# biointec/columba

Measured on AMD Instinct MI355X. Metric: reads/sec (150bp, k=4 edit, human ref), higher is better.
Workload: dtype u64; 1 GPU; synthetic human-like reference 3000 Mbp (GRCh38 is not available offline), 10000000 x 150 bp reads per GPU, k=4 edit distance, ALL mode, multiple_opt schemes with dynamic selection, dynamic partitioning, in-text switch 4, SA sparseness 4; reads_per_gpu=10000000, read_len=150, k=4, genome_bp=3000000000, index_bytes_hbm=24766778153, parallelism=read-shard x1, occurrences=33415092

## Files before the change

### columba_amd/csrc/columba_amd.hip

```cpp
#include "../../include/columba_amd.h"
#include "host_sam.hpp"
#include "host_schemes.hpp"
#include "kernels.hpp"
#include "dev_sam.hpp"

#include <chrono>
#include <cstring>
#include <functional>
#include <memory>
#include <mutex>
#include <thread>
#include <string>
#include <vector>

using namespace cmb;

static thread_local std::string g_err;
static int fail(int code, const std::string& msg) {
    g_err = msg;
    return code;
}
namespace cmb {
int failWith(int code, const std::string& msg) { return fail(code, msg); }
}
// ... 551 lines not shown

struct KernelTime {
    const char* name;
    float ms;
};

struct cmb_batch {
    cmb_index* ix = nullptr;
    uint32_t k = 0, nReads = 0, maxLen = 0, gw = 0;
    uint32_t minLen = 0;
    int metric = 1;
    DevStrategyK hostStrat{};
    bool wide = false;
    bool wideEdit = false;
    bool geoX = false;
    bool noSmallMatrix = false;
    DevStrategyKT<MAXP_WIDE> hostStratW{};
    DevBuf<DevStrategyKT<MAXP_WIDE>> stratW;
    DevBuf<PartOutT<MAXP_WIDE>> partsW;
    uint32_t sNumParts = 0, sPartition = 0, sNSchemes = 0, sMaxSearches = 0;
    hipStream_t stream = nullptr;
    DevBuf<uint8_t> reads, seq;
    DevBuf<uint32_t> rec;
    DevBuf<uint4> exr;
    DevBuf<uint8_t> psel;
    uint32_t recW = 0;
    DevBuf<uint64_t> offs;
    DevBuf<uint32_t> G;
    DevBuf<uint4> mfull;
    DevBuf<DevStrategyK> strat;
    DevBuf<uint4> bfsQ[2], bfsEv[2], bfsF, bfsC, bfsA;
    DevBuf<uint32_t> bfsCnt;
    DevBuf<unsigned long long> bfsBlockCnt;
    size_t bfsQCap = 0, bfsEvCap = 0, bfsFCap = 0, bfsCCap = 0, bfsACap = 0;
    DevBuf<uint4> nvQ[2];
    DevBuf<uint32_t> nvCnt;
    size_t nvQCap = 0;
    bool hasNaive = false;
    DevBuf<PartOut> parts;
    DevBuf<DfsTask> dfs;
    DevBuf<uint64_t> vW;
    DevBuf<uint4> tbq;
    DevBuf<uint8_t> dpSlab;
    DevBuf<uint32_t> dpList, dpWork;
    DevBuf<uint4> items;
    DevBuf<FMOccRec> fm, fmUniq;
    DevBuf<TextOccRec> text;
// ... 159 lines not shown
            minLen = std::min<uint32_t>(minLen, (uint32_t)(offs[i + 1] - offs[i]));
        }
        b->minLen = n_reads ? minLen : 0u;
        if (maxLen > (uint32_t)MAX_READ)
            return fail(CMB_ERR_UNSUPPORTED, "reads longer than " + std::to_string(MAX_READ) + " are not supported");
        maxLen = (maxLen + 15u) & ~15u;
        b->maxLen = maxLen;
        b->gw = gWords(maxLen);
        b->hostOffs.assign(offs, offs + n_reads + 1);
        HIPCHK(hipStreamCreateWithFlags(&b->stream, hipStreamNonBlocking));
        b->reads.uploadPadded((const uint8_t*)seqs, offs[n_reads], 64);
        b->offs.upload(offs, n_reads + 1);
        b->seq.alloc((size_t)2 * n_reads * maxLen);
        b->G.alloc((size_t)n_reads * 8 * b->gw);
        b->recW = ((1 + 2 * ((maxLen + 31) / 32)) + 3) / 4 * 4;
        b->rec.alloc((size_t)2 * n_reads * b->recW);
        if (b->wide) {
            b->stratW.upload(&b->hostStratW, 1);
            b->partsW.alloc((size_t)2 * n_reads);
        } else {
            b->strat.upload(&b->hostStrat, 1);
            b->parts.alloc((size_t)2 * n_reads);
        }
        b->dfs.alloc((size_t)n_reads * 2 + 4096);
        b->items.alloc((size_t)n_reads * 64 + 4096);
        b->fm.alloc((size_t)n_reads * 8 + 4096);
        b->text.alloc((size_t)n_reads * 48 + 4096);
        b->cnt.alloc(8);
        b->counters.alloc(CMB_CNT_MAX);
        *out = b.release();
        return CMB_OK;
    } catch (const std::exception& e) {
        return fail(CMB_ERR_DEVICE, e.what());
    }
}

namespace {

struct Timer {
    hipStream_t s;
    hipEvent_t a, b;
    std::vector<KernelTime>& out;
    Timer(hipStream_t st, std::vector<KernelTime>& o) : s(st), out(o) {
        (void)hipEventCreate(&a);
        (void)hipEventCreate(&b);
    }
    ~Timer() {
        (void)hipEventDestroy(a);
// ... 203 lines not shown
            HIPCHK(hipStreamSynchronize(s));
            memset(hcnt, 0, sizeof(hcnt));
            hcnt[0] = (uint32_t)b->presetItems.size();
            q.items = b->items.p;
            q.itemCap = (uint32_t)std::min<size_t>(b->items.n, 0xFFFFFFF0u);
        }
        int bfsAttempts = 0;
        for (int attempt = 0; !preset; attempt++) {
            HIPCHK(hipMemsetAsync(b->cnt.p, 0, 8 * sizeof(uint32_t), s));
            if (attempt) {
                HIPCHK(hipMemsetAsync(b->counters.p, 0, CMB_CNT_MAX * sizeof(unsigned long long), s));
            }
            q.items = b->items.p;
            q.itemCap = (uint32_t)std::min<size_t>(b->items.n, 0xFFFFFFF0u);
            q.fm = b->fm.p;
            q.fmCap = (uint32_t)std::min<size_t>(b->fm.n, 0xFFFFFFF0u);
            q.text = b->text.p;
            q.textCap = (uint32_t)std::min<size_t>(b->text.n, 0xFFFFFFF0u);
            const uint32_t dfsCap = (uint32_t)std::min<size_t>(b->dfs.n, 0xFFFFFFF0u);
            tm.begin();
            const uint32_t pParts = b->k ? b->sNumParts : 1;
            const uint32_t stratBytes = (uint32_t)(((b->wide ? sizeof(DevStrategyKT<MAXP_WIDE>) : sizeof(DevStrategyK)) + 15) / 16 * 16);
            const uint32_t rdWords = 2 * ((b->maxLen + 31) / 32);
            uint32_t nSlots = 1;
            const bool longReads = b->maxLen > 256;
            if (b->k) {
                if (b->exr.n < (size_t)pParts * tasks) {
                    b->exr.alloc((size_t)pParts * tasks);
                    b->psel.alloc(tasks);
                }
                const size_t pLds = stratBytes + (5 * pParts + rdWords) * 256 * sizeof(uint32_t);
                if (b->wide) {
                    constexpr int W = MAXP_WIDE;
                    auto kp = longReads ? (b->sPartition == 0 ? k_parts<0, true, W> : b->sPartition == 1 ? k_parts<1, true, W> : k_parts<2, true, W>)
                                        : (b->sPartition == 0 ? k_parts<0, false, W> : b->sPartition == 1 ? k_parts<1, false, W> : k_parts<2, false, W>);
                    if (pLds > 64 * 1024) HIPCHK(hipFuncSetAttribute((const void*)kp, hipFuncAttributeMaxDynamicSharedMemorySize, (int)pLds));
                    hipLaunchKernelGGL(kp, dim3(pSlots / 256), dim3(256), pLds, s, ix->d, b->stratW.p, nReads, b->k, b->maxLen, b->seq.p,
                                       (const uint4*)b->rec.p, b->recW / 4, b->partsW.p, b->exr.p, b->psel.p, q);
                } else {
                    auto kp = longReads ? (b->sPartition == 0 ? k_parts<0, true> : b->sPartition == 1 ? k_parts<1, true> : k_parts<2, true>)
                                        : (b->sPartition == 0 ? k_parts<0, false> : b->sPartition == 1 ? k_parts<1, false> : k_parts<2, false>);
                    hipLaunchKernelGGL(kp, dim3(pSlots / 256), dim3(256), pLds, s, ix->d, b->strat.p, nReads,
                                   b->k, b->maxLen, b->seq.p, (const uint4*)b->rec.p, b->recW / 4, b->parts.p, b->exr.p,
                                   b->psel.p, q);
                }
                nSlots = b->sMaxSearches + 1;
            }
            const uint64_t eTasks = (uint64_t)tasks * nSlots;
            const uint32_t eSlots = (uint32_t)std::min<uint64_t>(((eTasks + 255) / 256) * 256, 256ull * 4096ull);
            const size_t eLds = stratBytes + (pParts + rdWords) * 256 * sizeof(uint32_t);
            if (b->wide)
                hipLaunchKernelGGL((longReads ? k_exact<true, MAXP_WIDE> : k_exact<false, MAXP_WIDE>), dim3(eSlots / 256), dim3(256), eLds, s, ix->d,
                                   b->stratW.p, nReads, b->k, b->maxLen, nSlots, b->seq.p, (const uint4*)b->rec.p, b->recW / 4, b->partsW.p,
                                   b->exr.p, b->psel.p, b->dfs.p, dfsCap, q);
            else
                hipLaunchKernelGGL(longReads ? k_exact<true> : k_exact<false>, dim3(eSlots / 256), dim3(256), eLds,
                               s, ix->d, b->strat.p, nReads, b->k, b->maxLen, nSlots, b->seq.p, (const uint4*)b->rec.p,
                               b->recW / 4, b->parts.p, b->exr.p, b->psel.p, b->dfs.p, dfsCap, q);
            tm.end("k_partition");
            HIPCHK(hipGetLastError());
            HIPCHK(hipMemcpyAsync(hcnt, b->cnt.p, sizeof(hcnt), hipMemcpyDeviceToHost, s));
            HIPCHK(hipStreamSynchronize(s));
            uint32_t flags = hcnt[3];
            b->hasNaive = (flags & FLAG_UNSUPPORTED_READ) != 0;
            if (b->hasNaive) {
                tm.begin();
                const uint32_t maxPassN = b->maxLen + 2 * b->k + 4;
                if (!b->nvQCap) b->nvQCap = getenv("CMB_TEST_SMALL_POOLS") ? 64 : 16384;
                for (int j = 0; j < 2; j++)
                    if (b->nvQ[j].n < 3 * b->nvQCap) b->nvQ[j].alloc(3 * b->nvQCap);
                const size_t cntWords = (size_t)maxPassN + 2;
                if (b->nvCnt.n < cntWords) b->nvCnt.alloc(cntWords);
                HIPCHK(hipMemsetAsync(b->nvCnt.p, 0, cntWords * sizeof(uint32_t), s));
                NaiveBufs N{};
                N.Q[0] = b->nvQ[0].p;
                N.Q[1] = b->nvQ[1].p;
                N.qCap = (uint32_t)std::min<size_t>(b->nvQ[0].n / 3, 0xFFFFFFF0u);
                N.nq = b->nvCnt.p;
                const bool edit = b->metric == CMB_METRIC_EDIT;
                hipLaunchKernelGGL(k_naive_start, dim3((tasks + 255) / 256), dim3(256), 0, s, ix->d, b->psel.p, b->offs.p, tasks,
                                   b->k, edit ? 0u : 1u, N, q, b->geoX ? 1u : 0u);
// ... 12 lines not shown
                    HIPCHK(hipStreamSynchronize(s));
                    if (hcnt[3] & (FLAG_NAIVE_Q | FLAG_ITEM_OVERFLOW | FLAG_FMOCC_OVERFLOW)) break;
                    drained = hc[pass] == 0;
                }
                for (uint32_t p2 = 0; p2 <= pass && p2 < cntWords; p2++) peakQ = std::max(peakQ, hc[p2]);
                if (verbose) fprintf(stderr, "[naive] %u roots, %u passes, peak frontier %u\n", hc[0], pass, peakQ);
                tm.end("k_naive");
                HIPCHK(hipGetLastError());
                flags = hcnt[3];
                if (flags & FLAG_NAIVE_Q) {
                    if (attempt >= 60) return fail(CMB_ERR_INTERNAL, "the naive search's frontier keeps overflowing");
                    b->nvQCap = std::max<size_t>(4 * b->nvQCap, (size_t)peakQ + peakQ / 4);
                    continue;
                }
                if (!drained && !(flags & (FLAG_ITEM_OVERFLOW | FLAG_FMOCC_OVERFLOW)))
                    return fail(CMB_ERR_INTERNAL, "the naive search did not finish within its pass bound");
            }
            if (flags & FLAG_SEED_OVERLAP)
                return fail(CMB_ERR_INVALID,
                            "dynamic partitioning: the seeds of a read overlap — the k-mer size of the index is too large "
                            "for the seeding positions of this search strategy at this read length (the reference caps "
                            "the k-mer size, e.g. at 4 for kuch2 and 01*0: alignparameters.cpp:1070-1114, :1275-1278)");
            const uint32_t nDfs = hcnt[5];
            if (!(flags & (FLAG_ITEM_OVERFLOW | FLAG_DFS_OVERFLOW)) && nDfs) {
                tm.begin();
                if (b->metric == CMB_METRIC_EDIT) {
                    const uint32_t maxPass = 2 * b->maxLen + 8 * (b->wide ? MAXP_WIDE : MAXP) + 64;
                    const size_t qPlanes = 3 + (b->wide ? GeoW::PK_U4 : GeoN::PK_U4), evU4 = 1 + (b->wide ? GeoW::PK_U4 : GeoN::PK_U4);
                    if (!b->bfsQCap) {
                        const size_t slack = getenv("CMB_TEST_SMALL_POOLS") ? 64 : 65536;
                        const size_t per = getenv("CMB_TEST_SMALL_POOLS") ? 0 : 1;
                        b->bfsQCap = per * (size_t)nReads * 2 + slack;
                        b->bfsEvCap = per * (size_t)nReads / 2 + slack;
                        b->bfsFCap = per * (size_t)nReads * 16 + slack;
                        b->bfsCCap = per * (size_t)nReads * 2 + slack;
                        b->bfsACap = per * (size_t)nReads * 8 + slack;
                    }
                    b->bfsQCap = std::max<size_t>(b->bfsQCap, (size_t)nDfs + 1024);
                    for (int j = 0; j < 2; j++) {
                        if (b->bfsQ[j].n < qPlanes * b->bfsQCap) b->bfsQ[j].alloc(qPlanes * b->bfsQCap);
                        if (b->bfsEv[j].n < evU4 * b->bfsEvCap) b->bfsEv[j].alloc(evU4 * b->bfsEvCap);
                    }
                    if (b->bfsF.n < F_U4 * b->bfsFCap) b->bfsF.alloc(F_U4 * b->bfsFCap);
                    const uint32_t ctxU4 = b->geoX ? CTX_U4_X : ctxU4For(b->maxLen);
                    if (b->bfsC.n < (size_t)ctxU4 * b->bfsCCap) b->bfsC.alloc((size_t)ctxU4 * b->bfsCCap);
                    if (b->bfsA.n < b->bfsACap) b->bfsA.alloc(b->bfsACap);
                    const size_t cntWords = 2 * ((size_t)maxPass + 2) + 4;
// ... 142 lines not shown
                    for (uint32_t p2 = 0; p2 <= pass && p2 < cntWords; p2++) peakQ = std::max(peakQ, hc[p2]);
                    if (getenv("CMB_VERBOSE")) fprintf(stderr, "[hbfs] %u tasks, %u passes, peak frontier %u\n", nDfs, pass, peakQ);
                    BfsBufs Bf{};
                    Bf.blockCnt = b->bfsBlockCnt.p;
                    hipLaunchKernelGGL(k_bfs_finish, dim3(1), dim3(256), 0, s, Bf, q);
                    if (hcnt[3] & FLAG_BFS_Q) {
                        if (++bfsAttempts >= 24) return fail(CMB_ERR_INTERNAL, "frontier keeps overflowing");
                        b->bfsQCap = std::max<size_t>(2 * b->bfsQCap, (size_t)peakQ + peakQ / 4);
                        HIPCHK(hipStreamSynchronize(s));
                        tm.end("k_dfs");
                        continue;
                    }
                    if (!drained && !(hcnt[3] & BFS_STOP))
                        return fail(CMB_ERR_INTERNAL, "frontier search did not finish within its pass bound");
                }
                tm.end("k_dfs");
                HIPCHK(hipGetLastError());
                HIPCHK(hipMemcpyAsync(hcnt, b->cnt.p, sizeof(hcnt), hipMemcpyDeviceToHost, s));
                HIPCHK(hipStreamSynchronize(s));
                flags = hcnt[3];
            }
            if (flags & FLAG_CAPACITY)
                return fail(CMB_ERR_INTERNAL, "device search capacity exceeded (band width / descendants / stack)");
            if (flags & (FLAG_ITEM_OVERFLOW | FLAG_FMOCC_OVERFLOW | FLAG_DFS_OVERFLOW)) {
                if (attempt >= 60) return fail(CMB_ERR_INTERNAL, "work queues keep overflowing");
                const size_t grow = b->hasNaive ? 8 : 2;
                if (hcnt[0] > q.itemCap) b->items.alloc((size_t)hcnt[0] * grow + 1024);
                if (hcnt[1] > q.fmCap) b->fm.alloc((size_t)hcnt[1] * grow + 1024);
                if (hcnt[5] > dfsCap) b->dfs.alloc((size_t)hcnt[5] + hcnt[5] / 8 + 1024);
                continue;
            }
            break;
        }
        const uint32_t nItems = hcnt[0], nFm = hcnt[1];
        lap("prep + search");

        uint32_t nFmUniq = 0;
        if (nFm) {
            if (b->fmKeysA.n < nFm) {
                b->fmKeysA.alloc((size_t)nFm + nFm / 4 + 256);
                b->fmKeysB.alloc(b->fmKeysA.n);
                b->fmIdxA.alloc(b->fmKeysA.n);
                b->fmIdxB.alloc(b->fmKeysA.n);
                b->fmUniq.alloc(b->fmKeysA.n);
            }
            if (b->fmN.n < 1) b->fmN.alloc(1);
            HIPCHK(hipMemsetAsync(b->fmN.p, 0, sizeof(uint32_t), s));
            hipLaunchKernelGGL(k_fm_keys, dim3((nFm + 255) / 256), dim3(256), 0, s, b->fm.p, nFm, b->fmKeysA.p, b->fmIdxA.p);
            size_t tmpBytes = 0;
            HIPCHK(rocprim::radix_sort_pairs(nullptr, tmpBytes, b->fmKeysA.p, b->fmKeysB.p, b->fmIdxA.p, b->fmIdxB.p, nFm, 0,
                                             64, s));
            if (b->sortTmp.n < tmpBytes) b->sortTmp.alloc(tmpBytes + 256);
// ... 1635 lines not shown
```

### columba_amd/csrc/dev_partition.hpp

```cpp
#pragma once
#include "dev_search.hpp"

namespace cmb {

struct DfsTask {
    uint32_t rsId;
    uint8_t scheme, search, idx, pad;
    RangePair r;
    uint32_t depth;
};

template <int MP> struct PartOutT {
    uint16_t pb[MP], pe[MP];
};
typedef PartOutT<MAXP> PartOut;

enum : int { PH_CALC = 0, PH_DYN, PH_SEED, PH_FIN, PH_DONE };
enum : int { RQ_NONE = 0, RQ_RANK, RQ_SEED, RQ_REC };

template <int PARTITION, int MP = MAXP>
struct PartMachine {
    const DevIndex& ix;
    const DevStrategyKT<MP>& st;
    uint32_t rsId = 0, len = 0, k = 0;
    const uint8_t* seq = nullptr;
    uint32_t* lds;
    uint32_t ltid;
    uint32_t lstride;
    uint32_t lparts;
    __device__ __forceinline__ uint32_t& L(int field, int part) const {
        return lds[((uint32_t)field * lparts + (uint32_t)part) * lstride + ltid];
    }
    __device__ __forceinline__ uint32_t PB(int i) const { return L(4, i) & 0xFFFFu; }
    __device__ __forceinline__ uint32_t PE(int i) const { return L(4, i) >> 16; }
    __device__ __forceinline__ void setPB(int i, uint32_t v) { L(4, i) = (L(4, i) & 0xFFFF0000u) | (v & 0xFFFFu); }
    __device__ __forceinline__ void setPE(int i, uint32_t v) { L(4, i) = (L(4, i) & 0xFFFFu) | (v << 16); }
    __device__ __forceinline__ void setPBE(int i, uint32_t b, uint32_t e) { L(4, i) = (b & 0xFFFFu) | (e << 16); }
    __device__ __forceinline__ RangePair EX(int i) const {
        return RangePair{{L(0, i), L(1, i)}, {L(2, i), L(3, i)}};
    }
    __device__ __forceinline__ void setEX(int i, const RangePair& r) {
        L(0, i) = r.sa.b;
        L(1, i) = r.sa.e;
        L(2, i) = r.rev.b;
        L(3, i) = r.rev.e;
    }
    __device__ __forceinline__ uint32_t EXW(int i) const {
        const uint32_t b = L(0, i), e = L(1, i);
        return e <= b ? 0u : e - b;
    }
    uint32_t cNode = 0, cExp = 0, flags = 0;
    int phase = PH_DONE;
    int numParts = 0;
    int pi = 0;
    uint32_t ci = 0;
    uint32_t cend = 0;
    uint32_t cb = 0, ce = 0;
    int cdir = 0;
    uint32_t j = 0;
    int partToExtend = 0, dynDir = 0;
    int req = RQ_NONE;
    int reqMode = 0;
    uint32_t reqCode = 0;
    RangePair reqParent;

    __device__ PartMachine(const DevIndex& i, const DevStrategyKT<MP>& s, uint32_t* ldsBase, uint32_t tid, uint32_t stride)
        : ix(i), st(s), lds(ldsBase), ltid(tid), lstride(stride), lparts(s.numParts ? s.numParts : 1) {}
    __device__ void setReadWords(uint32_t maxLen) {
        rdBase = 5u * lparts;
        pw1 = (maxLen + 31) / 32;
    }

    uint32_t rdBase = 0, pw1 = 1;
    bool hasN = false;
// ... 247 lines not shown
            }
            return;
        }
    }

    __device__ void resume(bool ok, const RangePair& child) {
        cExp++;
        if (ok) cNode++;
        const RangePair res = ok ? child : RangePair{{0, 0}, {0, 0}};
        switch (phase) {
        case PH_CALC:
            setEX(pi < numParts ? pi : numParts - 1, res);
            if (ok) ci++;
            else ci = cend;
            break;
        case PH_DYN:
            setEX(partToExtend, res);
            break;
        default:
            break;
        }
    }

    __device__ void finish(PartOutT<MP>* parts, uint4* exr, uint8_t* psel, uint32_t total) {
        int sel = 0;
        if (st.nSchemes > 1) {
            uint32_t tot = 0;
            for (int i = 0; i < numParts; i++) tot += EXW(i);
            if (tot > (uint32_t)numParts) {
                uint32_t minValue = EXW(st.sch[0].critical);
                for (int i = 1; i < st.nSchemes; i++) {
                    const uint32_t w = EXW(st.sch[i].critical);
                    if (w < minValue) {
                        minValue = w;
                        sel = i;
                    }
                }
            }
        }
        PartOutT<MP> po;
#pragma unroll
        for (int i = 0; i < MP; i++) {
            po.pb[i] = i < numParts ? (uint16_t)PB(i) : (uint16_t)0;
            po.pe[i] = i < numParts ? (uint16_t)PE(i) : (uint16_t)0;
        }
        parts[rsId] = po;
        for (int i = 0; i < numParts; i++) {
            const RangePair r = EX(i);
            exr[(size_t)i * total + rsId] = make_uint4(r.sa.b, r.sa.e, r.rev.b, r.rev.e);
        }
        psel[rsId] = (uint8_t)sel;
        phase = PH_DONE;
    }
};

enum : int { EX_IDLE = 0, EX_HDR, EX_LOAD, EX_RUN, EX_K0 };

template <int MP = MAXP>
struct ExactLane {
    const DevIndex& ix;
    const DevStrategyKT<MP>& st;
    uint32_t* lds;
    uint32_t ltid, lstride, lparts, pw1;
    __device__ __forceinline__ uint32_t& PBE(int i) const { return lds[(uint32_t)i * lstride + ltid]; }
    __device__ __forceinline__ uint32_t PB(int i) const { return PBE(i) & 0xFFFFu; }
    __device__ __forceinline__ uint32_t PE(int i) const { return PBE(i) >> 16; }
    __device__ __forceinline__ uint32_t& RD(uint32_t plane, uint32_t w) const {
        return lds[(lparts + plane * pw1 + w) * lstride + ltid];
    }
    uint32_t rsId = 0, slot = 0, len = 0;
    const uint8_t* seq = nullptr;
    bool hasN = false;
    int phase = EX_IDLE;
    int sel = 0, partInSearch = 0;
    uint32_t ci = 0, exactLength = 0, k0i = 0;
// ... 29 lines not shown
        stR = r;
        stDepth = depth;
    }
    template <bool LONG>
    __device__ __forceinline__ void takeRecord(const uint4 v[5], const uint4* recBase, uint32_t recQ) {
        const uint32_t* vw = reinterpret_cast<const uint32_t*>(v);
        len = vw[0] & 0xFFFFu;
        hasN = (vw[0] >> 16) & 1u;
#pragma unroll
        for (uint32_t w = 0; w < 8; w++)
            if (w < pw1) {
                RD(0, w) = vw[1 + 2 * w];
                RD(1, w) = vw[2 + 2 * w];
            }
        if (LONG && pw1 > 8) {
            const uint32_t* recWords = reinterpret_cast<const uint32_t*>(recBase + (size_t)rsId * recQ);
            for (uint32_t w = 8; w < pw1; w++) {
                RD(0, w) = recWords[1 + 2 * w];
                RD(1, w) = recWords[2 + 2 * w];
            }
        }
    }

    __device__ void startSearch(const RangePair& first) {
        const DevSearchT<MP>& s = st.sch[sel].s[slot];
        cur = first;
        if (cur.width() <= ix.switchPoint) {
            phase = EX_IDLE;
            return;
        }
        const int f = s.order[0];
        partInSearch = 1;
        exactLength = PE(f) - PB(f);
        ci = 0;
        phase = EX_RUN;
    }

    __device__ void advance() {
        const DevSearchT<MP>& s = st.sch[sel].s[slot];
        for (;;) {
            if (s.U[partInSearch] == 0) {
                const int part = s.order[partInSearch];
                const uint32_t b = PB(part), e = PE(part);
                const uint32_t n = e > b ? e - b : 0;
                if (ci < n) {
                    const uint32_t c = code(s.dir[partInSearch] == 0 ? b + ci : e - ci - 1);
                    if (c >= 1 && c <= 4) {
                        const bool uni = s.uniAll || partInSearch >= (int)s.uniIdx;
                        req = true;
                        reqMode = uni ? 2 : (s.dir[partInSearch] == 0 ? 0 : 1);
                        reqCode = c;
                        return;
                    }
                    cur = RangePair{{0, 0}, {0, 0}};
// ... 62 lines not shown
```

### columba_amd/csrc/dev_search.hpp

```cpp
#pragma once
#include "dev_index.hpp"
#include "dev_matrix.hpp"

namespace cmb {

constexpr int MAXP = 8;
constexpr int MAXP_WIDE = 16;
constexpr int MAXS = 16;
constexpr int MAXSCH = 4;
constexpr int MAX_READ = 480;
constexpr int DESC_MAX = 56;

template <int MP> struct DevSearchT {
    uint8_t n;
    uint8_t order[MP], L[MP], U[MP], dir[MP], dsw[MP];
    uint8_t low[MP], high[MP];
    uint8_t uniAll, uniIdx;
};
template <int MP> struct DevSchemeT {
    uint8_t nSearches, critical;
    DevSearchT<MP> s[MAXS];
};
template <int MP> struct DevStrategyKT {
    uint8_t metric, partition, numParts, nSchemes;
// ... 4 lines not shown
    DevSchemeT<MP> sch[MAXSCH];
};
typedef DevSearchT<MAXP> DevSearch;
typedef DevSchemeT<MAXP> DevScheme;
typedef DevStrategyKT<MAXP> DevStrategyK;

enum { ITEM_EDIT = 0, ITEM_HAMMING = 1, ITEM_EXACT = 2 };
__device__ __forceinline__ uint32_t packMeta(uint32_t shift, uint32_t maxED, uint32_t minED, uint32_t fixed,
                                             uint32_t kind) {
    return (shift & 0xFFFu) | (maxED << 12) | (minED << 16) | (fixed << 20) | (kind << 21);
}
struct FMOccRec {
    uint32_t rsId, b, e, depth, dist, shift;
};
struct TextOccRec {
    uint32_t rsId, begin, end, dist;
};

enum : uint32_t { FLAG_ITEM_OVERFLOW = 1, FLAG_FMOCC_OVERFLOW = 2, FLAG_TEXT_OVERFLOW = 4, FLAG_CAPACITY = 8,
                  FLAG_UNSUPPORTED_READ = 16, FLAG_DFS_OVERFLOW = 32, FLAG_TRACE_RULE = 64,
                  FLAG_BFS_Q = 128, FLAG_BFS_EV = 256, FLAG_BFS_F = 512, FLAG_BFS_CTX = 1024, FLAG_BFS_ARENA = 2048,
                  FLAG_SEED_OVERLAP = 4096,
                  FLAG_NAIVE_Q = 8192,
                  FLAG_NARROW_MATRIX = 16384 };
constexpr uint32_t FLAG_BITS[] = {FLAG_ITEM_OVERFLOW, FLAG_FMOCC_OVERFLOW, FLAG_TEXT_OVERFLOW, FLAG_CAPACITY,
                                  FLAG_UNSUPPORTED_READ, FLAG_DFS_OVERFLOW, FLAG_TRACE_RULE, FLAG_BFS_Q, FLAG_BFS_EV,
                                  FLAG_BFS_F, FLAG_BFS_CTX, FLAG_BFS_ARENA, FLAG_SEED_OVERLAP, FLAG_NAIVE_Q, FLAG_NARROW_MATRIX};
constexpr bool flagBitsDisjoint() {
    uint32_t seen = 0;
    for (uint32_t b : FLAG_BITS) {
        if (b == 0 || (b & (b - 1)) != 0 || (seen & b) != 0) return false;
        seen |= b;
    }
    return true;
}
static_assert(flagBitsDisjoint(), "every flag is one bit of its own");

struct KeyBits {
    uint32_t group, begin, dist, distMask, wMask;
};
__host__ __device__ __forceinline__ KeyBits keyBits(uint32_t layout) {
    return layout == 2u ? KeyBits{42u, 10u, 6u, 15u, 31u} : layout == 1u ? KeyBits{40u, 8u, 4u, 15u, 0u} : KeyBits{40u, 8u, 5u, 7u, 15u};
}

struct Queues {
    uint4* items;
    uint32_t itemCap;
    FMOccRec* fm;
    uint32_t fmCap;
    TextOccRec* text;
// ... 7 lines not shown
```

### columba_amd/csrc/kernels.hpp

```cpp
#pragma once
#include "dev_partition.hpp"
#include <cstring>
#include <rocprim/device/device_radix_sort.hpp>
#include <rocprim/device/device_scan.hpp>
#include <rocprim/device/device_run_length_encode.hpp>

namespace cmb {

__global__ void k_rank(DevIndex ix, int rev, const uint32_t* __restrict__ c, const uint64_t* __restrict__ p,
                       uint64_t n, uint64_t* __restrict__ out) {
    const uint64_t i = (uint64_t)blockIdx.x * blockDim.x + threadIdx.x;
    if (i >= n) return;
    out[i] = rank1(rev ? ix.rev : ix.fwd, c[i], p[i]);
}

__device__ __forceinline__ uint32_t rank9RefLayout(const uint64_t* bv, const uint64_t* cnt, uint64_t nWords, uint64_t p) {
    uint64_t w = p >> 6, b = p & 63;
    if (nWords == 0) return 0;
    if (w >= nWords) {
        w = nWords - 1;
        b = 64;
    }
    uint64_t rv = cnt[(w >> 3) * 2];
    const uint32_t sub = (uint32_t)(w & 7u);
// ... 257 lines not shown
    loadRankPairRaw(t, tr.b, tr.e, v);
}
__device__ __forceinline__ bool takeExtend(const DevIndex& ix, int mode, const RangePair& parent, uint32_t code,
                                           const uint4 v[4], RangePair& child) {
    DevBWT t = ix.fwd;
    Range tr = parent.sa;
    if (mode == 0) {
        t = ix.rev;
        tr = parent.rev;
    }
    uint32_t Rb[4], Re[4];
    uint4 w[2];
    rankPairEnd(v, tr.b, tr.e, w);
    ranksFromRaw(v, tr.b, t.dollarPos, Rb);
    ranksFromRaw(w, tr.e, t.dollarPos, Re);
    return childFromRanks(ix, mode, parent, code, Rb, Re, tr.b > t.dollarPos ? 1u : 0u, tr.e > t.dollarPos ? 1u : 0u,
                          child);
}

template <int PARTITION, bool LONG, int MP = MAXP>
__global__ void __launch_bounds__(256, MP == MAXP ? 4 : 2)
k_parts(DevIndex ix, const DevStrategyKT<MP>* __restrict__ stp, uint32_t nReads, uint32_t k, uint32_t maxLen,
        const uint8_t* __restrict__ seq, const uint4* __restrict__ rec, uint32_t recQ, PartOutT<MP>* __restrict__ parts,
        uint4* __restrict__ exr, uint8_t* __restrict__ psel, Queues q) {
    typedef DevStrategyKT<MP> DevStrategyK;
    extern __shared__ uint32_t partLds[];
    constexpr uint32_t STRAT_WORDS = (uint32_t)((sizeof(DevStrategyK) + 15) / 16 * 4);
    for (uint32_t i = threadIdx.x; i < sizeof(DevStrategyK) / 4; i += blockDim.x)
        partLds[i] = reinterpret_cast<const uint32_t*>(stp)[i];
    __syncthreads();
    const DevStrategyK& lst = *reinterpret_cast<const DevStrategyK*>(partLds);
    PartMachine<PARTITION, MP> m(ix, lst, partLds + STRAT_WORDS, threadIdx.x, blockDim.x);
    m.setReadWords(maxLen);
    const uint32_t total = 2 * nReads;
    const uint32_t stride = gridDim.x * blockDim.x;
    const uint32_t first = blockIdx.x * blockDim.x + threadIdx.x;
    for (uint32_t base = first & ~63u; base < total; base += stride) {
        const uint32_t rs = base + (threadIdx.x & 63u);
        uint4 v[MP];
        m.phase = PH_DONE;
        m.req = RQ_NONE;
        if (rs < total) {
#pragma unroll
            for (uint32_t j = 0; j < 5; j++)
                if (j < recQ) v[j] = rec[(size_t)rs * recQ + j];
            m.template begin<LONG>(rs, v, rec, recQ, seq + (size_t)rs * maxLen, k);
            if (m.phase == PH_DONE) psel[rs] = 0x80u;
        }
        if (__ballot(m.req == RQ_SEED) != 0ull) {
            if (m.req == RQ_SEED) {
                m.seedIssue(v);
                m.req = RQ_NONE;
                m.seedTake(v);
            }
        }
        for (;;) {
            if (m.req == RQ_NONE) m.advance();
            if (__ballot(m.req == RQ_RANK) == 0ull) break;
            if (m.req == RQ_RANK) {
                uint4 rk[4];
                issueExtend(ix, m.reqMode, m.reqParent, rk);
                RangePair child;
                const bool ok = takeExtend(ix, m.reqMode, m.reqParent, m.reqCode, rk, child);
                m.req = RQ_NONE;
                m.resume(ok, child);
            }
        }
        if (m.phase == PH_FIN) m.finish(parts, exr, psel, total);
    }
    const uint32_t local[2] = {m.cNode, m.cExp};
    const int which[2] = {0, 7};
    flushCounters(q, local, which, 2);
    if (m.flags) atomicOr(&q.cnt[3], m.flags);
}

template <bool LONG, int MP = MAXP>
__global__ void __launch_bounds__(256, MP == MAXP ? 4 : 2)
k_exact(DevIndex ix, const DevStrategyKT<MP>* __restrict__ stp, uint32_t nReads, uint32_t k, uint32_t maxLen,
        uint32_t nSlots, const uint8_t* __restrict__ seq, const uint4* __restrict__ rec, uint32_t recQ,
        const PartOutT<MP>* __restrict__ parts, const uint4* __restrict__ exr, const uint8_t* __restrict__ psel,
        DfsTask* __restrict__ dfsQ, uint32_t dfsCap, Queues q) {
    typedef DevStrategyKT<MP> DevStrategyK;
    typedef DevSchemeT<MP> DevScheme;
    extern __shared__ uint32_t partLds[];
    constexpr uint32_t STRAT_WORDS = (uint32_t)((sizeof(DevStrategyK) + 15) / 16 * 4);
    for (uint32_t i = threadIdx.x; i < sizeof(DevStrategyK) / 4; i += blockDim.x)
        partLds[i] = reinterpret_cast<const uint32_t*>(stp)[i];
    __syncthreads();
    const DevStrategyK& lst = *reinterpret_cast<const DevStrategyK*>(partLds);
    ExactLane<MP> m(ix, lst, partLds + STRAT_WORDS, threadIdx.x, blockDim.x, maxLen);
    const uint32_t total = 2 * nReads;
    const uint64_t nTasks = (uint64_t)total * nSlots;
    uint64_t nextT = (uint64_t)blockIdx.x * blockDim.x + threadIdx.x;
    const int numParts = lst.numParts;
    const uint32_t sw = ix.switchPoint;
    bool done = false, ovI = false, ovD = false;
    WaveChunk chI, chD;
    auto holeI = [&](uint32_t i) { q.items[i] = make_uint4(0xFFFFFFFFu, 0, 0, 0); };
    auto holeD = [&](uint32_t i) { dfsQ[i].rsId = 0xFFFFFFFFu; };
    for (;;) {
        if (!done && m.phase == EX_IDLE && !m.req) {
            if (nextT >= nTasks) done = true;
            else {
                m.rsId = (uint32_t)(nextT / nSlots);
                m.slot = (uint32_t)(nextT % nSlots);
                m.seq = seq + (size_t)m.rsId * maxLen;
                m.phase = k == 0 ? EX_LOAD : EX_HDR;
                nextT += (uint64_t)gridDim.x * blockDim.x;
            }
        }
        if (!done && !m.req) {
            if (m.phase == EX_RUN) m.advance();
            else if (m.phase == EX_K0) m.advanceK0();
        }
        uint4 v[MP];
        uint32_t hdr = 0;
        const int ph = done ? EX_IDLE : m.phase;
        const bool isPost = m.slot == nSlots - 1;
        if (m.req) {
            issueExtend(ix, m.reqMode, m.cur, v);
        } else if (ph == EX_HDR) {
            hdr = psel[m.rsId];
            const uint4* pp = reinterpret_cast<const uint4*>(parts + m.rsId);
#pragma unroll
            for (int j = 0; j < MP / 4; j++) v[j] = pp[j];
        } else if (ph == EX_LOAD) {
            if (k == 0 || !isPost) {
#pragma unroll
                for (uint32_t j = 0; j < 5; j++)
                    if (j < recQ) v[j] = rec[(size_t)m.rsId * recQ + j];
                if (k != 0) v[5] = exr[(size_t)lst.sch[m.sel].s[m.slot].order[0] * total + m.rsId];
            } else {
#pragma unroll
                for (int i = 0; i < MP; i++)
                    if (i < numParts) v[i] = exr[(size_t)i * total + m.rsId];
            }
        }
        if (m.req) {
            RangePair child;
            const bool ok = takeExtend(ix, m.reqMode, m.cur, m.reqCode, v, child);
            m.req = false;
            m.resume(ok, child);
        } else if (ph == EX_HDR) {
            m.sel = (int)(hdr & 0x7Fu);
            const uint16_t* pv = reinterpret_cast<const uint16_t*>(v);
#pragma unroll
            for (int i = 0; i < MP; i++)
                if (i < numParts) m.PBE(i) = (uint32_t)pv[i] | ((uint32_t)pv[MP + i] << 16);
            m.phase = EX_LOAD;
            if (hdr & 0x80u) m.phase = EX_IDLE;
            else if (!isPost) {
                const DevScheme& sch = lst.sch[m.sel];
                if (m.slot >= sch.nSearches) m.phase = EX_IDLE;
                else if (sch.s[m.slot].U[0] > 0) {
                    if (lst.metric == 1) m.cStart++;
                    m.emitDfs(0, RangePair{{0, ix.n}, {0, ix.n}}, 0);
                    m.phase = EX_IDLE;
                }
            }
        } else if (ph == EX_LOAD) {
            if (k == 0) {
                m.template takeRecord<LONG>(v, rec, recQ);
                m.cur = RangePair{{0, ix.n}, {0, 0}};
                m.k0i = m.len;
                m.phase = m.len == 0 ? EX_IDLE : EX_K0;
            } else if (!isPost) {
                m.template takeRecord<LONG>(v, rec, recQ);
                m.startSearch(RangePair{{v[5].x, v[5].y}, {v[5].z, v[5].w}});
            } else {
                m.phase = EX_IDLE;
            }
        }
        if (__ballot(ph == EX_LOAD && k != 0 && isPost) != 0ull) {
            const bool mine = ph == EX_LOAD && k != 0 && isPost;
#pragma unroll
            for (int i = 0; i < MP; i++) {
                if (i >= numParts) break;
                uint32_t n = 0, a = 0, meta = 0;
                if (mine) {
                    const uint32_t width = v[i].y > v[i].x ? v[i].y - v[i].x : 0u;
                    if (width != 0 && width <= sw) {
                        n = width;
                        const uint32_t bg = m.PB(i);
                        if (lst.metric == 1) {
                            m.cImm++;
                            a = bg == 0 ? 0 : bg + k;
                            meta = packMeta(0, k, 0, bg == 0, ITEM_EDIT);
                        } else {
                            a = bg;
                            meta = packMeta(0, k, 0, 0, ITEM_HAMMING);
                        }
                    }
                }
                if (__ballot(n > 0) == 0ull) continue;
                const uint32_t o = chI.alloc(&q.cnt[0], q.itemCap, n, 256u, ovI, holeI);
                if (n && o != 0xFFFFFFFFu)
                    for (uint32_t t = 0; t < n; t++) q.items[o + t] = make_uint4(m.rsId, v[i].x + t, a, meta);
            }
        }
        if (__ballot(m.stN > 0) != 0ull) {
            const uint32_t o = chI.alloc(&q.cnt[0], q.itemCap, m.stN, 256u, ovI, holeI);
            if (m.stN && o != 0xFFFFFFFFu)
                for (uint32_t t = 0; t < m.stN; t++) q.items[o + t] = make_uint4(m.rsId, m.stB + t, m.stA, m.stMeta);
            m.stN = 0;
        }
        if (__ballot(m.stDfs) != 0ull) {
            const uint32_t o = chD.alloc(&q.cnt[5], dfsCap, m.stDfs ? 1u : 0u, 64u, ovD, holeD);
            if (m.stDfs && o != 0xFFFFFFFFu) {
                DfsTask t;
                t.rsId = m.rsId;
                t.scheme = (uint8_t)m.sel;
                t.search = (uint8_t)m.slot;
                t.idx = (uint8_t)m.stIdx;
                t.pad = 0;
                t.r = m.stR;
                t.depth = m.stDepth;
                dfsQ[o] = t;
            }
            m.stDfs = false;
        }
// ... 1644 lines not shown
```

Before: 58.59 million reads/s.

## Emit exact-phase tasks from partition kernel into compact queue instead of dense slots

```diff
diff --git a/columba_amd/csrc/columba_amd.hip b/columba_amd/csrc/columba_amd.hip
--- a/columba_amd/csrc/columba_amd.hip
+++ b/columba_amd/csrc/columba_amd.hip
@@ -597,7 +597,7 @@
     hipStream_t stream = nullptr;
     DevBuf<uint8_t> reads, seq;
     DevBuf<uint32_t> rec;
-    DevBuf<uint4> exr;
+    DevBuf<ExactTask> exq;
     DevBuf<uint8_t> psel;
     uint32_t recW = 0;
     DevBuf<uint64_t> offs;
@@ -803,8 +803,10 @@
             b->strat.upload(&b->hostStrat, 1);
             b->parts.alloc((size_t)2 * n_reads);
         }
-        b->dfs.alloc((size_t)n_reads * 2 + 4096);
-        b->items.alloc((size_t)n_reads * 64 + 4096);
+        const bool smallPools = getenv("CMB_TEST_SMALL_POOLS") != nullptr;
+        b->dfs.alloc(smallPools ? 64 : (size_t)n_reads * 2 + 4096);
+        b->items.alloc(smallPools ? 64 : (size_t)n_reads * 64 + 4096);
+        b->exq.alloc(smallPools ? 16 : 65536);
         b->fm.alloc((size_t)n_reads * 8 + 4096);
         b->text.alloc((size_t)n_reads * 48 + 4096);
         b->cnt.alloc(8);
@@ -1054,13 +1056,10 @@
             const uint32_t pParts = b->k ? b->sNumParts : 1;
             const uint32_t stratBytes = (uint32_t)(((b->wide ? sizeof(DevStrategyKT<MAXP_WIDE>) : sizeof(DevStrategyK)) + 15) / 16 * 16);
             const uint32_t rdWords = 2 * ((b->maxLen + 31) / 32);
-            uint32_t nSlots = 1;
             const bool longReads = b->maxLen > 256;
+            const uint32_t exCap = (uint32_t)std::min<size_t>(b->exq.n, 0xFFFFFFF0u);
             if (b->k) {
-                if (b->exr.n < (size_t)pParts * tasks) {
-                    b->exr.alloc((size_t)pParts * tasks);
-                    b->psel.alloc(tasks);
-                }
+                if (b->psel.n < tasks) b->psel.alloc(tasks);
                 const size_t pLds = stratBytes + (5 * pParts + rdWords) * 256 * sizeof(uint32_t);
                 if (b->wide) {
                     constexpr int W = MAXP_WIDE;
@@ -1068,27 +1067,25 @@
                                         : (b->sPartition == 0 ? k_parts<0, false, W> : b->sPartition == 1 ? k_parts<1, false, W> : k_parts<2, false, W>);
                     if (pLds > 64 * 1024) HIPCHK(hipFuncSetAttribute((const void*)kp, hipFuncAttributeMaxDynamicSharedMemorySize, (int)pLds));
                     hipLaunchKernelGGL(kp, dim3(pSlots / 256), dim3(256), pLds, s, ix->d, b->stratW.p, nReads, b->k, b->maxLen, b->seq.p,
-                                       (const uint4*)b->rec.p, b->recW / 4, b->partsW.p, b->exr.p, b->psel.p, q);
+                                       (const uint4*)b->rec.p, b->recW / 4, b->partsW.p, b->psel.p, b->dfs.p, dfsCap, b->exq.p, exCap, q);
                 } else {
                     auto kp = longReads ? (b->sPartition == 0 ? k_parts<0, true> : b->sPartition == 1 ? k_parts<1, true> : k_parts<2, true>)
                                         : (b->sPartition == 0 ? k_parts<0, false> : b->sPartition == 1 ? k_parts<1, false> : k_parts<2, false>);
                     hipLaunchKernelGGL(kp, dim3(pSlots / 256), dim3(256), pLds, s, ix->d, b->strat.p, nReads,
-                                   b->k, b->maxLen, b->seq.p, (const uint4*)b->rec.p, b->recW / 4, b->parts.p, b->exr.p,
-                                   b->psel.p, q);
+                                   b->k, b->maxLen, b->seq.p, (const uint4*)b->rec.p, b->recW / 4, b->parts.p, b->psel.p,
+                                   b->dfs.p, dfsCap, b->exq.p, exCap, q);
                 }
-                nSlots = b->sMaxSearches + 1;
-            }
-            const uint64_t eTasks = (uint64_t)tasks * nSlots;
-            const uint32_t eSlots = (uint32_t)std::min<uint64_t>(((eTasks + 255) / 256) * 256, 256ull * 4096ull);
+            }
+            const uint32_t eSlots = b->k ? 256u * 256u : (uint32_t)std::min<uint64_t>((((uint64_t)tasks + 255) / 256) * 256, 256ull * 4096ull);
             const size_t eLds = stratBytes + (pParts + rdWords) * 256 * sizeof(uint32_t);
             if (b->wide)
                 hipLaunchKernelGGL((longReads ? k_exact<true, MAXP_WIDE> : k_exact<false, MAXP_WIDE>), dim3(eSlots / 256), dim3(256), eLds, s, ix->d,
-                                   b->stratW.p, nReads, b->k, b->maxLen, nSlots, b->seq.p, (const uint4*)b->rec.p, b->recW / 4, b->partsW.p,
-                                   b->exr.p, b->psel.p, b->dfs.p, dfsCap, q);
+                                   b->stratW.p, nReads, b->k, b->maxLen, b->seq.p, (const uint4*)b->rec.p, b->recW / 4, b->partsW.p,
+                                   b->exq.p, exCap, b->dfs.p, dfsCap, q);
             else
                 hipLaunchKernelGGL(longReads ? k_exact<true> : k_exact<false>, dim3(eSlots / 256), dim3(256), eLds,
-                               s, ix->d, b->strat.p, nReads, b->k, b->maxLen, nSlots, b->seq.p, (const uint4*)b->rec.p,
-                               b->recW / 4, b->parts.p, b->exr.p, b->psel.p, b->dfs.p, dfsCap, q);
+                               s, ix->d, b->strat.p, nReads, b->k, b->maxLen, b->seq.p, (const uint4*)b->rec.p,
+                               b->recW / 4, b->parts.p, b->exq.p, exCap, b->dfs.p, dfsCap, q);
             tm.end("k_partition");
             HIPCHK(hipGetLastError());
             HIPCHK(hipMemcpyAsync(hcnt, b->cnt.p, sizeof(hcnt), hipMemcpyDeviceToHost, s));
@@ -1147,7 +1144,8 @@
                             "for the seeding positions of this search strategy at this read length (the reference caps "
                             "the k-mer size, e.g. at 4 for kuch2 and 01*0: alignparameters.cpp:1070-1114, :1275-1278)");
             const uint32_t nDfs = hcnt[5];
-            if (!(flags & (FLAG_ITEM_OVERFLOW | FLAG_DFS_OVERFLOW)) && nDfs) {
+            if (verbose && b->k) fprintf(stderr, "[prologue] %u items, %u search tasks, %u searches with further exact phases\n", hcnt[0], nDfs, hcnt[4]);
+            if (!(flags & (FLAG_ITEM_OVERFLOW | FLAG_DFS_OVERFLOW | FLAG_EXACT_OVERFLOW)) && nDfs) {
                 tm.begin();
                 if (b->metric == CMB_METRIC_EDIT) {
                     const uint32_t maxPass = 2 * b->maxLen + 8 * (b->wide ? MAXP_WIDE : MAXP) + 64;
@@ -1336,12 +1334,16 @@
             }
             if (flags & FLAG_CAPACITY)
                 return fail(CMB_ERR_INTERNAL, "device search capacity exceeded (band width / descendants / stack)");
-            if (flags & (FLAG_ITEM_OVERFLOW | FLAG_FMOCC_OVERFLOW | FLAG_DFS_OVERFLOW)) {
+            if (flags & (FLAG_ITEM_OVERFLOW | FLAG_FMOCC_OVERFLOW | FLAG_DFS_OVERFLOW | FLAG_EXACT_OVERFLOW)) {
                 if (attempt >= 60) return fail(CMB_ERR_INTERNAL, "work queues keep overflowing");
+                if (verbose)
+                    fprintf(stderr, "[retry] queues too small:%s%s%s%s\n", hcnt[0] > q.itemCap ? " items" : "", hcnt[1] > q.fmCap ? " occurrences" : "",
+                            hcnt[5] > dfsCap ? " tasks" : "", hcnt[4] > exCap ? " exact" : "");
                 const size_t grow = b->hasNaive ? 8 : 2;
                 if (hcnt[0] > q.itemCap) b->items.alloc((size_t)hcnt[0] * grow + 1024);
                 if (hcnt[1] > q.fmCap) b->fm.alloc((size_t)hcnt[1] * grow + 1024);
                 if (hcnt[5] > dfsCap) b->dfs.alloc((size_t)hcnt[5] + hcnt[5] / 8 + 1024);
+                if (hcnt[4] > exCap) b->exq.alloc((size_t)hcnt[4] + hcnt[4] / 8 + 1024);
                 continue;
             }
             break;
diff --git a/columba_amd/csrc/dev_partition.hpp b/columba_amd/csrc/dev_partition.hpp
--- a/columba_amd/csrc/dev_partition.hpp
+++ b/columba_amd/csrc/dev_partition.hpp
@@ -9,6 +9,14 @@
     RangePair r;
     uint32_t depth;
 };
+
+struct alignas(16) ExactTask {
+    uint32_t rsId;
+    uint8_t scheme, search, pad[2];
+    uint32_t pad2[2];
+    RangePair r;
+};
+static_assert(sizeof(ExactTask) == 32, "k_exact loads an ExactTask as two 16-byte words");
 
 template <int MP> struct PartOutT {
     uint16_t pb[MP], pe[MP];
@@ -49,7 +57,7 @@
         const uint32_t b = L(0, i), e = L(1, i);
         return e <= b ? 0u : e - b;
     }
-    uint32_t cNode = 0, cExp = 0, flags = 0;
+    uint32_t cNode = 0, cExp = 0, cImm = 0, cStart = 0, flags = 0;
     int phase = PH_DONE;
     int numParts = 0;
     int pi = 0;
@@ -343,7 +351,7 @@
         }
     }
 
-    __device__ void finish(PartOutT<MP>* parts, uint4* exr, uint8_t* psel, uint32_t total) {
+    __device__ int finish(PartOutT<MP>* parts, uint8_t* psel) {
         int sel = 0;
         if (st.nSchemes > 1) {
             uint32_t tot = 0;
@@ -366,12 +374,43 @@
             po.pe[i] = i < numParts ? (uint16_t)PE(i) : (uint16_t)0;
         }
         parts[rsId] = po;
-        for (int i = 0; i < numParts; i++) {
-            const RangePair r = EX(i);
-            exr[(size_t)i * total + rsId] = make_uint4(r.sa.b, r.sa.e, r.rev.b, r.rev.e);
-        }
         psel[rsId] = (uint8_t)sel;
         phase = PH_DONE;
+        return sel;
+    }
+
+    __device__ void startSearches(int sel, uint32_t& dfsMask, uint32_t& exactMask) const {
+        const DevSchemeT<MP>& sch = st.sch[sel];
+        uint32_t dfs = 0, exact = 0;
+        for (uint32_t slot = 0; slot < sch.nSearches; slot++) {
+            const DevSearchT<MP>& s = sch.s[slot];
+            const bool whole = s.U[0] > 0;
+            const bool live = whole || EXW(s.order[0]) > ix.switchPoint;
+            const bool approx = whole || s.U[1] > 0;
+            const uint32_t bit = live ? 1u << slot : 0u;
+            dfs |= approx ? bit : 0u;
+            exact |= approx ? 0u : bit;
+        }
+        dfsMask = dfs;
+        exactMask = exact;
+    }
+    __device__ DfsTask dfsTask(int sel, uint32_t slot) const {
+        const DevSearchT<MP>& s = st.sch[sel].s[slot];
+        const bool whole = s.U[0] > 0;
+        const int f = s.order[0];
+        DfsTask t;
+        t.rsId = rsId;
+        t.scheme = (uint8_t)sel;
+        t.search = (uint8_t)slot;
+        t.idx = whole ? 0 : 1;
+        t.pad = 0;
+        t.r = whole ? RangePair{{0, ix.n}, {0, ix.n}} : EX(f);
+        t.depth = whole ? 0u : PE(f) - PB(f);
+        return t;
+    }
+    __device__ __forceinline__ uint32_t narrowWidth(int i) const {
+        const uint32_t w = EXW(i);
+        return w <= ix.switchPoint ? w : 0u;
     }
 };
 
@@ -447,14 +486,9 @@
         }
     }
 
-    __device__ void startSearch(const RangePair& first) {
-        const DevSearchT<MP>& s = st.sch[sel].s[slot];
+    __device__ void continueSearch(const RangePair& first) {
+        const int f = st.sch[sel].s[slot].order[0];
         cur = first;
-        if (cur.width() <= ix.switchPoint) {
-            phase = EX_IDLE;
-            return;
-        }
-        const int f = s.order[0];
         partInSearch = 1;
         exactLength = PE(f) - PB(f);
         ci = 0;
diff --git a/columba_amd/csrc/dev_search.hpp b/columba_amd/csrc/dev_search.hpp
--- a/columba_amd/csrc/dev_search.hpp
+++ b/columba_amd/csrc/dev_search.hpp
@@ -50,10 +50,12 @@
                   FLAG_BFS_Q = 128, FLAG_BFS_EV = 256, FLAG_BFS_F = 512, FLAG_BFS_CTX = 1024, FLAG_BFS_ARENA = 2048,
                   FLAG_SEED_OVERLAP = 4096,
                   FLAG_NAIVE_Q = 8192,
-                  FLAG_NARROW_MATRIX = 16384 };
+                  FLAG_NARROW_MATRIX = 16384,
+                  FLAG_EXACT_OVERFLOW = 32768 };
 constexpr uint32_t FLAG_BITS[] = {FLAG_ITEM_OVERFLOW, FLAG_FMOCC_OVERFLOW, FLAG_TEXT_OVERFLOW, FLAG_CAPACITY,
                                   FLAG_UNSUPPORTED_READ, FLAG_DFS_OVERFLOW, FLAG_TRACE_RULE, FLAG_BFS_Q, FLAG_BFS_EV,
-                                  FLAG_BFS_F, FLAG_BFS_CTX, FLAG_BFS_ARENA, FLAG_SEED_OVERLAP, FLAG_NAIVE_Q, FLAG_NARROW_MATRIX};
+                                  FLAG_BFS_F, FLAG_BFS_CTX, FLAG_BFS_ARENA, FLAG_SEED_OVERLAP, FLAG_NAIVE_Q, FLAG_NARROW_MATRIX,
+                                  FLAG_EXACT_OVERFLOW};
 constexpr bool flagBitsDisjoint() {
     uint32_t seen = 0;
     for (uint32_t b : FLAG_BITS) {
diff --git a/columba_amd/csrc/kernels.hpp b/columba_amd/csrc/kernels.hpp
--- a/columba_amd/csrc/kernels.hpp
+++ b/columba_amd/csrc/kernels.hpp
@@ -303,7 +303,8 @@
 __global__ void __launch_bounds__(256, MP == MAXP ? 4 : 2)
 k_parts(DevIndex ix, const DevStrategyKT<MP>* __restrict__ stp, uint32_t nReads, uint32_t k, uint32_t maxLen,
         const uint8_t* __restrict__ seq, const uint4* __restrict__ rec, uint32_t recQ, PartOutT<MP>* __restrict__ parts,
-        uint4* __restrict__ exr, uint8_t* __restrict__ psel, Queues q) {
+        uint8_t* __restrict__ psel, DfsTask* __restrict__ dfsQ, uint32_t dfsCap, ExactTask* __restrict__ exQ, uint32_t exCap,
+        Queues q) {
     typedef DevStrategyKT<MP> DevStrategyK;
     extern __shared__ uint32_t partLds[];
     constexpr uint32_t STRAT_WORDS = (uint32_t)((sizeof(DevStrategyK) + 15) / 16 * 4);
@@ -314,6 +315,11 @@
     PartMachine<PARTITION, MP> m(ix, lst, partLds + STRAT_WORDS, threadIdx.x, blockDim.x);
     m.setReadWords(maxLen);
     const uint32_t total = 2 * nReads;
+    bool ovI = false, ovD = false, ovE = false;
+    WaveChunk chI, chD, chE;
+    auto holeI = [&](uint32_t i) { q.items[i] = make_uint4(0xFFFFFFFFu, 0, 0, 0); };
+    auto holeD = [&](uint32_t i) { dfsQ[i].rsId = 0xFFFFFFFFu; };
+    auto holeE = [&](uint32_t i) { exQ[i].rsId = 0xFFFFFFFFu; };
     const uint32_t stride = gridDim.x * blockDim.x;
     const uint32_t first = blockIdx.x * blockDim.x + threadIdx.x;
     for (uint32_t base = first & ~63u; base < total; base += stride) {
@@ -347,22 +353,81 @@
                 m.resume(ok, child);
             }
         }
-        if (m.phase == PH_FIN) m.finish(parts, exr, psel, total);
-    }
-    const uint32_t local[2] = {m.cNode, m.cExp};
-    const int which[2] = {0, 7};
-    flushCounters(q, local, which, 2);
+        const bool fin = m.phase == PH_FIN;
+        int sel = 0;
+        uint32_t dfsMask = 0, exactMask = 0, nItems = 0;
+        if (fin) {
+            sel = m.finish(parts, psel);
+            m.startSearches(sel, dfsMask, exactMask);
+            for (int i = 0; i < m.numParts; i++) nItems += m.narrowWidth(i);
+        }
+        {
+            uint32_t o = chI.alloc(&q.cnt[0], q.itemCap, nItems, 1u, ovI, holeI);
+            if (nItems) {
+                for (int i = 0; i < m.numParts; i++) {
+                    const uint32_t n = m.narrowWidth(i);
+                    if (!n) continue;
+                    const uint32_t bg = m.PB(i), row = m.EX(i).sa.b;
+                    uint32_t a, meta;
+                    if (lst.metric == 1) {
+                        m.cImm++;
+                        a = bg == 0 ? 0 : bg + k;
+                        meta = packMeta(0, k, 0, bg == 0, ITEM_EDIT);
+                    } else {
+                        a = bg;
+                        meta = packMeta(0, k, 0, 0, ITEM_HAMMING);
+                    }
+                    if (o != 0xFFFFFFFFu)
+                        for (uint32_t t = 0; t < n; t++) q.items[o++] = make_uint4(m.rsId, row + t, a, meta);
+                }
+            }
+        }
+        {
+            uint32_t o = chD.alloc(&q.cnt[5], dfsCap, (uint32_t)__popc(dfsMask), 1u, ovD, holeD);
+            if (lst.metric == 1) m.cStart += (uint32_t)__popc(dfsMask);
+            if (o != 0xFFFFFFFFu)
+                for (uint32_t mk = dfsMask; mk; mk &= mk - 1u) dfsQ[o++] = m.dfsTask(sel, (uint32_t)__ffs((int)mk) - 1u);
+        }
+        {
+            uint32_t o = chE.alloc(&q.cnt[4], exCap, (uint32_t)__popc(exactMask), 1u, ovE, holeE);
+            if (o != 0xFFFFFFFFu)
+                for (uint32_t mk = exactMask; mk; mk &= mk - 1u) {
+                    const uint32_t slot = (uint32_t)__ffs((int)mk) - 1u;
+                    ExactTask t;
+                    t.rsId = m.rsId;
+                    t.scheme = (uint8_t)sel;
+                    t.search = (uint8_t)slot;
+                    t.pad[0] = t.pad[1] = 0;
+                    t.pad2[0] = t.pad2[1] = 0;
+                    t.r = m.EX(lst.sch[sel].s[slot].order[0]);
+                    exQ[o++] = t;
+                }
+        }
+    }
+    chI.fill(holeI);
+    chD.fill(holeD);
+    chE.fill(holeE);
+    if (ovI) m.flags |= FLAG_ITEM_OVERFLOW;
+    if (ovD) m.flags |= FLAG_DFS_OVERFLOW;
+    if (ovE) m.flags |= FLAG_EXACT_OVERFLOW;
+    const uint32_t local[4] = {m.cNode, m.cExp, m.cImm, m.cStart};
+    const int which[4] = {0, 7, 5, 6};
+    flushCounters(q, local, which, 4);
     if (m.flags) atomicOr(&q.cnt[3], m.flags);
 }
 
 template <bool LONG, int MP = MAXP>
 __global__ void __launch_bounds__(256, MP == MAXP ? 4 : 2)
 k_exact(DevIndex ix, const DevStrategyKT<MP>* __restrict__ stp, uint32_t nReads, uint32_t k, uint32_t maxLen,
-        uint32_t nSlots, const uint8_t* __restrict__ seq, const uint4* __restrict__ rec, uint32_t recQ,
-        const PartOutT<MP>* __restrict__ parts, const uint4* __restrict__ exr, const uint8_t* __restrict__ psel,
+        const uint8_t* __restrict__ seq, const uint4* __restrict__ rec, uint32_t recQ,
+        const PartOutT<MP>* __restrict__ parts, const ExactTask* __restrict__ exQ, uint32_t exCap,
         DfsTask* __restrict__ dfsQ, uint32_t dfsCap, Queues q) {
     typedef DevStrategyKT<MP> DevStrategyK;
-    typedef DevSchemeT<MP> DevScheme;
+    uint64_t nTasks = 2ull * nReads;
+    if (k != 0) {
+        nTasks = q.cnt[4];
+        if (nTasks == 0 || nTasks > exCap) return;
+    }
     extern __shared__ uint32_t partLds[];
     constexpr uint32_t STRAT_WORDS = (uint32_t)((sizeof(DevStrategyK) + 15) / 16 * 4);
     for (uint32_t i = threadIdx.x; i < sizeof(DevStrategyK) / 4; i += blockDim.x)
@@ -370,22 +435,23 @@
     __syncthreads();
     const DevStrategyK& lst = *reinterpret_cast<const DevStrategyK*>(partLds);
     ExactLane<MP> m(ix, lst, partLds + STRAT_WORDS, threadIdx.x, blockDim.x, maxLen);
-    const uint32_t total = 2 * nReads;
-    const uint64_t nTasks = (uint64_t)total * nSlots;
     uint64_t nextT = (uint64_t)blockIdx.x * blockDim.x + threadIdx.x;
+    uint32_t task = 0;
     const int numParts = lst.numParts;
-    const uint32_t sw = ix.switchPoint;
     bool done = false, ovI = false, ovD = false;
     WaveChunk chI, chD;
     auto holeI = [&](uint32_t i) { q.items[i] = make_uint4(0xFFFFFFFFu, 0, 0, 0); };
     auto holeD = [&](uint32_t i) { dfsQ[i].rsId = 0xFFFFFFFFu; };
+    constexpr int NV = MP > 5 + MP / 4 ? MP : 5 + MP / 4;
     for (;;) {
         if (!done && m.phase == EX_IDLE && !m.req) {
             if (nextT >= nTasks) done = true;
             else {
-                m.rsId = (uint32_t)(nextT / nSlots);
-                m.slot = (uint32_t)(nextT % nSlots);
-                m.seq = seq + (size_t)m.rsId * maxLen;
+                task = (uint32_t)nextT;
+                if (k == 0) {
+                    m.rsId = task;
+                    m.seq = seq + (size_t)m.rsId * maxLen;
+                }
                 m.phase = k == 0 ? EX_LOAD : EX_HDR;
                 nextT += (uint64_t)gridDim.x * blockDim.x;
             }
@@ -394,27 +460,22 @@
             if (m.phase == EX_RUN) m.advance();
             else if (m.phase == EX_K0) m.advanceK0();
         }
-        uint4 v[MP];
-        uint32_t hdr = 0;
+        uint4 v[NV];
         const int ph = done ? EX_IDLE : m.phase;
-        const bool isPost = m.slot == nSlots - 1;
         if (m.req) {
             issueExtend(ix, m.reqMode, m.cur, v);
         } else if (ph == EX_HDR) {
-            hdr = psel[m.rsId];
-            const uint4* pp = reinterpret_cast<const uint4*>(parts + m.rsId);
-#pragma unroll
-            for (int j = 0; j < MP / 4; j++) v[j] = pp[j];
+            const uint4* pt = reinterpret_cast<const uint4*>(exQ + task);
+            v[0] = pt[0];
+            v[1] = pt[1];
         } else if (ph == EX_LOAD) {
-            if (k == 0 || !isPost) {
-#pragma unroll
-                for (uint32_t j = 0; j < 5; j++)
-                    if (j < recQ) v[j] = rec[(size_t)m.rsId * recQ + j];
-                if (k != 0) v[5] = exr[(size_t)lst.sch[m.sel].s[m.slot].order[0] * total + m.rsId];
-            } else {
-#pragma unroll
-                for (int i = 0; i < MP; i++)
-                    if (i < numParts) v[i] = exr[(size_t)i * total + m.rsId];
+#pragma unroll
+            for (uint32_t j = 0; j < 5; j++)
+                if (j < recQ) v[j] = rec[(size_t)m.rsId * recQ + j];
+            if (k != 0) {
+                const uint4* pp = reinterpret_cast<const uint4*>(parts + m.rsId);
+#pragma unroll
+                for (int j = 0; j < MP / 4; j++) v[5 + j] = pp[j];
             }
         }
         if (m.req) {
@@ -423,60 +484,24 @@
             m.req = false;
             m.resume(ok, child);
         } else if (ph == EX_HDR) {
-            m.sel = (int)(hdr & 0x7Fu);
-            const uint16_t* pv = reinterpret_cast<const uint16_t*>(v);
-#pragma unroll
-            for (int i = 0; i < MP; i++)
-                if (i < numParts) m.PBE(i) = (uint32_t)pv[i] | ((uint32_t)pv[MP + i] << 16);
-            m.phase = EX_LOAD;
-            if (hdr & 0x80u) m.phase = EX_IDLE;
-            else if (!isPost) {
-                const DevScheme& sch = lst.sch[m.sel];
-                if (m.slot >= sch.nSearches) m.phase = EX_IDLE;
-                else if (sch.s[m.slot].U[0] > 0) {
-                    if (lst.metric == 1) m.cStart++;
-                    m.emitDfs(0, RangePair{{0, ix.n}, {0, ix.n}}, 0);
-                    m.phase = EX_IDLE;
-                }
-            }
+            m.rsId = v[0].x;
+            m.sel = (int)(v[0].y & 0xFFu);
+            m.slot = (v[0].y >> 8) & 0xFFu;
+            m.cur = RangePair{{v[1].x, v[1].y}, {v[1].z, v[1].w}};
+            m.seq = seq + (size_t)m.rsId * maxLen;
+            m.phase = m.rsId == 0xFFFFFFFFu ? EX_IDLE : EX_LOAD;
         } else if (ph == EX_LOAD) {
+            m.template takeRecord<LONG>(v, rec, recQ);
             if (k == 0) {
-                m.template takeRecord<LONG>(v, rec, recQ);
                 m.cur = RangePair{{0, ix.n}, {0, 0}};
                 m.k0i = m.len;
                 m.phase = m.len == 0 ? EX_IDLE : EX_K0;
-            } else if (!isPost) {
-                m.template takeRecord<LONG>(v, rec, recQ);
-                m.startSearch(RangePair{{v[5].x, v[5].y}, {v[5].z, v[5].w}});
             } else {
-                m.phase = EX_IDLE;
-            }
-        }
-        if (__ballot(ph == EX_LOAD && k != 0 && isPost) != 0ull) {
-            const bool mine = ph == EX_LOAD && k != 0 && isPost;
-#pragma unroll
-            for (int i = 0; i < MP; i++) {
-                if (i >= numParts) break;
-                uint32_t n = 0, a = 0, meta = 0;
-                if (mine) {
-                    const uint32_t width = v[i].y > v[i].x ? v[i].y - v[i].x : 0u;
-                    if (width != 0 && width <= sw) {
-                        n = width;
-                        const uint32_t bg = m.PB(i);
-                        if (lst.metric == 1) {
-                            m.cImm++;
-                            a = bg == 0 ? 0 : bg + k;
-                            meta = packMeta(0, k, 0, bg == 0, ITEM_EDIT);
-                        } else {
-                            a = bg;
-                            meta = packMeta(0, k, 0, 0, ITEM_HAMMING);
-                        }
-                    }
-                }
-                if (__ballot(n > 0) == 0ull) continue;
-                const uint32_t o = chI.alloc(&q.cnt[0], q.itemCap, n, 256u, ovI, holeI);
-                if (n && o != 0xFFFFFFFFu)
-                    for (uint32_t t = 0; t < n; t++) q.items[o + t] = make_uint4(m.rsId, v[i].x + t, a, meta);
+                const uint16_t* pv = reinterpret_cast<const uint16_t*>(v + 5);
+#pragma unroll
+                for (int i = 0; i < MP; i++)
+                    if (i < numParts) m.PBE(i) = (uint32_t)pv[i] | ((uint32_t)pv[MP + i] << 16);
+                m.continueSearch(m.cur);
             }
         }
         if (__ballot(m.stN > 0) != 0ull) {
```

New measurement: 61.23 million reads/s (median of 6 runs). 1.05x the previous value.
